# Melthizar/RRTE

Measured on AMD Instinct MI355X. Metric: Mray/s (primary+shadow) at 1920x1080, sdf-showcase scene; 1/2/4/8 GPU, higher is better.
Workload: dtype f32; 1 GPU; sdf-showcase 1920x1080, lambert_shadow, spp=1, max_depth=1, pixel-centre jitter; scene=sdf-showcase, width=1920, height=1080, mode=lambert_shadow, primary_rays_per_frame=2073600, frames_in_flight=4, hw_queues=32, parallelism=single

## Files before the change

### rrte_amd/abi.py

```python
from __future__ import annotations

import ctypes as C
import os
from pathlib import Path

import numpy as np

_HERE = Path(__file__).resolve().parent
LIB_PATH = Path(os.environ.get("RRTE_HIP_LIB", _HERE / "lib" / "librrte_hip.so"))

RRTE_OK, RRTE_INVALID_ARG, RRTE_HIP_ERROR, RRTE_RCCL_ERROR, RRTE_UNSUPPORTED_PRIM, RRTE_NO_DEVICE = range(6)
STATUS_NAMES = {0: "OK", 1: "INVALID_ARG", 2: "HIP_ERROR", 3: "RCCL_ERROR", 4: "UNSUPPORTED_PRIM", 5: "NO_DEVICE"}

PRIM_SPHERE, PRIM_PLANE, PRIM_TRIANGLE, PRIM_CUBE, PRIM_CYLINDER, PRIM_CONE, PRIM_CAPSULE, PRIM_SDF, PRIM_MESH = range(9)
PRIM_MESH_INSTANCE = 9
MAT_LAMBERTIAN, MAT_METAL, MAT_DIELECTRIC, MAT_EMISSIVE = range(4)
LIGHT_POINT, LIGHT_DIRECTIONAL, LIGHT_SPOT, LIGHT_AMBIENT = range(4)
PERSPECTIVE, ORTHOGRAPHIC = 0, 1
MODE_REFCOMPAT, MODE_LAMBERT_SHADOW = 0, 1
JITTER_CENTER, JITTER_RANDOM = 0, 1
ABI_VERSION = 2
FLAG_F32_LINEAR = 1
FLAG_GATHER_OVERLAP = 2

SDF_SPHERE, SDF_BOX, SDF_CYLINDER, SDF_PRISM, SDF_TORUS = 1, 2, 3, 4, 5
SDF_TUBE, SDF_RING, SDF_CONE, SDF_CAPSULE, SDF_ELLIPSOID = 6, 7, 8, 9, 10
SDF_UNION, SDF_DIFFERENCE, SDF_INTERSECTION = 32, 33, 34
SDF_SMOOTH_UNION, SDF_SMOOTH_DIFFERENCE, SDF_SMOOTH_INTERSECTION = 35, 36, 37
SDF_BEND, SDF_TWIST, SDF_TAPER, SDF_NOISE, SDF_WAVE = 64, 65, 66, 67, 68
SDF_POP_POINT = 96
SDF_MAX_STACK, SDF_MAX_POINT_STACK, SDF_MAX_OCTAVES = 8, 4, 8
UNIQUE_ID_BYTES = 128
JIT_OFF, JIT_ON, JIT_AUTO = 0, 1, 2
FPCHECK_SQRT, FPCHECK_RCP, FPCHECK_DIV, FPCHECK_SQRT_HW, FPCHECK_GAMMA_U8, FPCHECK_SQRT_BF = 0, 1, 2, 3, 4, 5


class Prim(C.Structure):
    _fields_ = [
        ("kind", C.c_uint32), ("material", C.c_int32), ("sdf_first", C.c_uint32), ("sdf_count", C.c_uint32),
        ("sdf_max_steps", C.c_uint32), ("sdf_step_scale", C.c_float), ("sdf_hit_eps", C.c_float),
        ("flags", C.c_uint32), ("p", C.c_float * 20), ("trs", C.c_float * 10), ("_pad", C.c_float * 10),
    ]


class Material(C.Structure):
    _fields_ = [("kind", C.c_uint32), ("fuzz", C.c_float), ("ior", C.c_float), ("_pad0", C.c_float),
                ("albedo", C.c_float * 4)]


class Light(C.Structure):
    _fields_ = [
        ("kind", C.c_uint32), ("intensity", C.c_float), ("range", C.c_float), ("linear", C.c_float),
        ("quadratic", C.c_float), ("inner_angle", C.c_float), ("outer_angle", C.c_float), ("_pad0", C.c_float),
        ("position", C.c_float * 4), ("direction", C.c_float * 4), ("color", C.c_float * 4),
    ]


class SdfNode(C.Structure):
    _fields_ = [("op", C.c_uint32), ("i", C.c_uint32 * 3), ("f", C.c_float * 12)]


class Camera(C.Structure):
    _fields_ = [
        ("position", C.c_float * 3), ("projection", C.c_uint32), ("rotation", C.c_float * 4),
        ("scale", C.c_float * 3), ("fov", C.c_float), ("aspect_ratio", C.c_float), ("near_plane", C.c_float),
        ("far_plane", C.c_float), ("left", C.c_float), ("right", C.c_float), ("bottom", C.c_float),
        ("top", C.c_float), ("_pad", C.c_float * 1),
    ]


class RenderParams(C.Structure):
    _fields_ = [
        ("width", C.c_uint32), ("height", C.c_uint32), ("samples_per_pixel", C.c_uint32),
        ("max_depth", C.c_uint32), ("mode", C.c_uint32), ("jitter", C.c_uint32), ("seed", C.c_uint32),
        ("flags", C.c_uint32), ("background", C.c_float * 4), ("t_min", C.c_float), ("shadow_bias", C.c_float),
        ("gamma", C.c_float), ("band_rows", C.c_uint32),
    ]


class MeshVertex(C.Structure):
    _fields_ = [("position", C.c_float * 3), ("normal", C.c_float * 3)]


class SceneIR(C.Structure):
    _fields_ = [
        ("prims", C.POINTER(Prim)), ("num_prims", C.c_uint32),
        ("materials", C.POINTER(Material)), ("num_materials", C.c_uint32),
        ("lights", C.POINTER(Light)), ("num_lights", C.c_uint32),
        ("sdf_nodes", C.POINTER(SdfNode)), ("num_sdf_nodes", C.c_uint32),
        ("camera", Camera),
        ("mesh_vertices", C.POINTER(MeshVertex)), ("num_mesh_vertices", C.c_uint32),
        ("mesh_indices", C.POINTER(C.c_uint32)), ("num_mesh_indices", C.c_uint32),
        ("mesh_version", C.c_uint64),
    ]


class Stats(C.Structure):
    _fields_ = [("primary_rays", C.c_uint64), ("shadow_rays", C.c_uint64), ("kernel_ms", C.c_double),
                ("gather_ms", C.c_double), ("upload_ms", C.c_double), ("frames", C.c_uint64),
                ("jit_active", C.c_uint32), ("hot_tiles", C.c_uint32), ("jit_compile_ms", C.c_double)]


assert C.sizeof(Prim) == 192 and C.sizeof(Material) == 32 and C.sizeof(Light) == 80
assert C.sizeof(SdfNode) == 64 and C.sizeof(Camera) == 80 and C.sizeof(RenderParams) == 64

_P = C.c_void_p
EXPORTS = {
    "rrte_hip_abi_version": (C.c_uint32, []),
    "rrte_hip_create": (C.c_int, [C.c_int, C.POINTER(_P)]),
    "rrte_hip_destroy": (None, [_P]),
    "rrte_hip_last_error": (C.c_char_p, [_P]),
    "rrte_hip_render": (C.c_int, [_P, C.POINTER(SceneIR), C.POINTER(RenderParams), _P]),
    "rrte_hip_render_f32": (C.c_int, [_P, C.POINTER(SceneIR), C.POINTER(RenderParams), _P, _P]),
    "rrte_hip_render_async": (C.c_int, [_P, C.POINTER(SceneIR), C.POINTER(RenderParams), _P, _P, _P]),
    "rrte_hip_synchronize": (C.c_int, [_P]),
    "rrte_hip_query": (C.c_int, [_P, C.POINTER(C.c_uint32)]),
    "rrte_hip_stats": (C.c_int, [_P, C.POINTER(Stats)]),
    "rrte_hip_set_jit": (C.c_int, [_P, C.c_int]),
    "rrte_hip_jit_check": (C.c_int, [C.POINTER(SceneIR), C.c_int, C.c_char_p, C.c_size_t]),
    "rrte_hip_fpcheck": (C.c_int, [C.c_int, C.c_int, C.c_uint64, C.c_uint64, C.POINTER(C.c_uint64)]),
    "rrte_hip_sdf_guards": (C.c_int, [C.POINTER(SdfNode), C.c_uint32, C.c_uint32, C.POINTER(SdfNode),
                                      C.POINTER(C.c_uint32)]),
    "rrte_hip_tile_order_plan": (C.c_int, [C.POINTER(C.c_uint32), C.c_uint32, C.c_uint32, C.POINTER(C.c_uint32),
                                           C.c_uint32, C.POINTER(C.c_uint32)]),
    "rrte_hip_jit_cache_key": (C.c_int, [C.c_char_p, C.c_char_p, C.c_char_p, C.c_size_t]),
    "rrte_hip_check_word": (C.c_int, [_P, C.POINTER(C.c_uint64)]),
    "rrte_hip_scene_dump": (C.c_int, [C.POINTER(SceneIR), C.POINTER(RenderParams), C.c_char_p]),
    "rrte_hip_scene_load": (C.c_int, [C.c_char_p, C.POINTER(SceneIR), C.POINTER(RenderParams), C.POINTER(_P)]),
    "rrte_hip_scene_free": (None, [_P]),
    "rrte_hip_comm_unique_id": (C.c_int, [_P]),
    "rrte_hip_comm_init": (C.c_int, [_P, C.c_int, C.c_int, _P]),
    "rrte_hip_render_gather": (C.c_int, [_P, C.POINTER(SceneIR), C.POINTER(RenderParams), C.c_int, _P]),
    "rrte_hip_render_gather_async": (C.c_int, [_P, C.POINTER(SceneIR), C.POINTER(RenderParams), C.c_int, _P, _P]),
    "rrte_hip_band_rows_for_rank": (C.c_uint32, [C.c_uint32, C.c_uint32, C.c_int, C.c_int]),
    "rrte_hip_band_layout": (C.c_int, [C.POINTER(SceneIR), C.POINTER(RenderParams), C.c_int, C.c_int,
                                       C.POINTER(C.c_uint32), C.POINTER(C.c_uint32), C.POINTER(C.c_uint32)]),
    "rrte_hip_band_rows_for_rank_ex": (C.c_uint32, [C.c_uint32, C.c_uint32, C.c_int, C.c_int, C.c_uint32, C.c_uint32,
                                                    C.c_uint32]),
    "rrte_hip_set_gather_batch": (C.c_int, [_P, C.c_uint32]),
    "rrte_hip_flush": (C.c_int, [_P]),
    "rrte_hip_gather_info": (C.c_int, [_P, C.POINTER(C.c_uint64), C.POINTER(C.c_uint32)]),
    "rrte_hip_build_id": (C.c_int, [C.c_char_p, C.c_size_t]),
    "rrte_hip_host_register": (C.c_int, [_P, C.c_void_p, C.c_size_t]),
    "rrte_hip_host_unregister": (C.c_int, [_P, C.c_void_p]),
    "rrte_hip_set_comm_timeout": (C.c_int, [_P, C.c_uint32]),
}

QUERY_CLOSEST, QUERY_ANY = 0, 1
QUERY_MAX_RAYS = 1 << 24


class Ray(C.Structure):
    _fields_ = [("origin", C.c_float * 3), ("t_min", C.c_float), ("direction", C.c_float * 3), ("t_max", C.c_float)]


class RayHit(C.Structure):
    _fields_ = [("t", C.c_float), ("prim", C.c_int32), ("point", C.c_float * 3), ("normal", C.c_float * 3),
                ("front_face", C.c_uint32), ("tri", C.c_uint32), ("material", C.c_int32), ("_pad", C.c_uint32)]


assert C.sizeof(Ray) == 32 and C.sizeof(RayHit) == 48

RAY_DTYPE = np.dtype([("origin", "<f4", (3,)), ("t_min", "<f4"), ("direction", "<f4", (3,)), ("t_max", "<f4")])
RAY_HIT_DTYPE = np.dtype([("t", "<f4"), ("prim", "<i4"), ("point", "<f4", (3,)), ("normal", "<f4", (3,)),
                          ("front_face", "<u4"), ("tri", "<u4"), ("material", "<i4"), ("_pad", "<u4")])
assert RAY_DTYPE.itemsize == 32 and RAY_HIT_DTYPE.itemsize == 48

QUERY_EXPORTS = {
    "rrte_hip_raycast": (C.c_int, [_P, C.POINTER(SceneIR), C.POINTER(Ray), C.c_uint32, C.c_uint32, C.POINTER(RayHit)]),
    "rrte_hip_raycast_async": (C.c_int, [_P, C.POINTER(SceneIR), _P, C.c_uint32, C.c_uint32, _P, _P]),
    "rrte_hip_pick": (C.c_int, [_P, C.POINTER(SceneIR), C.POINTER(RenderParams), C.POINTER(C.c_uint32), C.c_uint32,
                                C.POINTER(RayHit)]),
}

class MeshInfo(C.Structure):
    _fields_ = [("bvh_builds", C.c_uint64), ("ranges", C.c_uint32), ("tri_slots", C.c_uint32),
                ("bvh_nodes", C.c_uint32), ("_pad", C.c_uint32)]


assert C.sizeof(MeshInfo) == 24

MESH_EXPORTS = {
    "rrte_hip_mesh_info": (C.c_int, [_P, C.POINTER(MeshInfo)]),
}

class RefitInfo(C.Structure):
    _fields_ = [("refits", C.c_uint64), ("device_refits", C.c_uint64), ("levels", C.c_uint32),
                ("deformed", C.c_uint32)]


assert C.sizeof(RefitInfo) == 24

REFIT_EXPORTS = {
    "rrte_hip_mesh_refit": (C.c_int, [_P, C.POINTER(SceneIR)]),
    "rrte_hip_refit_info": (C.c_int, [_P, C.POINTER(RefitInfo)]),
    "rrte_hip_mesh_nodes": (C.c_int, [_P, C.c_void_p, C.c_size_t, C.POINTER(C.c_uint32)]),
    "rrte_hip_mesh_slots": (C.c_int, [_P, C.POINTER(C.c_uint32), C.c_size_t, C.POINTER(C.c_uint32)]),
}

MESH_BUILD_HOST, MESH_BUILD_DEVICE = 0, 1


class BuildInfo(C.Structure):
    _fields_ = [("device_builds", C.c_uint64), ("host_fallbacks", C.c_uint64), ("policy", C.c_uint32),
                ("depth", C.c_uint32)]


assert C.sizeof(BuildInfo) == 24

BUILD_EXPORTS = {
    "rrte_hip_set_mesh_build": (C.c_int, [_P, C.c_uint32]),
    "rrte_hip_build_info": (C.c_int, [_P, C.POINTER(BuildInfo)]),
}

SCENE_ACCEL_OFF, SCENE_ACCEL_ON = 0, 1
ACCEL_COUNT = 1
ACCEL_DEFAULT_MIN_PRIMS, ACCEL_MAX_PRIMS = 65, 16384


class AccelInfo(C.Structure):
    _fields_ = [("builds", C.c_uint64), ("fallbacks", C.c_uint64), ("searches", C.c_uint64),
                ("candidates", C.c_uint64), ("policy", C.c_uint32), ("min_prims", C.c_uint32),
                ("flags", C.c_uint32), ("nodes", C.c_uint32), ("depth", C.c_uint32), ("bounded", C.c_uint32),
                ("unbounded", C.c_uint32), ("reserved", C.c_uint32)]


assert C.sizeof(AccelInfo) == 64

ACCEL_EXPORTS = {
    "rrte_hip_set_scene_accel": (C.c_int, [_P, C.c_uint32, C.c_uint32, C.c_uint32]),
    "rrte_hip_accel_info": (C.c_int, [_P, C.POINTER(AccelInfo)]),
}

ENTRY_NONE, ENTRY_GENERIC, ENTRY_GENERAL, ENTRY_PLAIN = 0, 1, 2, 3

JIT_EXPORTS = {
    "rrte_hip_jit_entry": (C.c_int, [_P, C.POINTER(C.c_uint32)]),
    "rrte_hip_tile_rects": (C.c_int, [C.POINTER(SceneIR), C.POINTER(RenderParams), C.POINTER(C.c_uint32),
                                      C.POINTER(C.c_uint32), C.POINTER(C.c_uint32)]),
}

_lib = None


def load() -> C.CDLL:
    global _lib
    if _lib is not None:
        return _lib
    if not LIB_PATH.exists():
        raise RuntimeError(
            f"librrte_hip.so not found at {LIB_PATH}; build it with `python -c 'import __graft_entry__ as g; g.build()'`"
        )
    try:
        import torch
    except Exception:
        pass
    lib = C.CDLL(str(LIB_PATH), mode=C.RTLD_GLOBAL)
    for name, (res, args) in {**EXPORTS, **QUERY_EXPORTS, **MESH_EXPORTS, **REFIT_EXPORTS, **BUILD_EXPORTS,
                               **ACCEL_EXPORTS, **JIT_EXPORTS}.items():
        fn = getattr(lib, name)
        fn.restype = res
        fn.argtypes = args
    if lib.rrte_hip_abi_version() != ABI_VERSION:
        raise RuntimeError("librrte_hip.so ABI version mismatch")
    _lib = lib
    return lib


class RrteError(RuntimeError):
    def __init__(self, status: int, msg: str):
        super().__init__(f"rrte_hip {STATUS_NAMES.get(status, status)}: {msg}")
        self.status = status


def band_layout(scene_ref, params_ref, nranks: int, root: int = 0) -> tuple:
    sky, rb, pb = C.c_uint32(), C.c_uint32(), C.c_uint32()
    st = load().rrte_hip_band_layout(scene_ref, params_ref, nranks, root, C.byref(sky), C.byref(rb), C.byref(pb))
    if st != RRTE_OK:
        raise RuntimeError(f"rrte_hip_band_layout: status {st}")
    return sky.value, rb.value, pb.value


def build_id() -> str:
    buf = C.create_string_buffer(64)
    st = load().rrte_hip_build_id(buf, 64)
    if st != RRTE_OK:
        raise RuntimeError(f"rrte_hip_build_id: status {st}")
    return buf.value.decode()
```

### rrte_amd/csrc/jit.hip

```cpp
#include <hip/hip_runtime.h>
#include <hip/hiprtc.h>

#include <chrono>
#include <cinttypes>
#include <cstdio>
#include <cstdlib>
#include <cstring>
#include <mutex>
#include <sys/stat.h>
#include <unistd.h>
#include <string>
#include <vector>

#include "jit.hpp"

namespace rrte {
namespace {

struct JitHeader {
    const char* name;
    const char* text;
};
#include "jit_headers.inc"

void emit_f(std::string& s, float v) {
    char buf[48];
    if (v != v) {
        snprintf(buf, sizeof buf, "__builtin_nanf(\"\")");
    } else if (v == __builtin_huge_valf()) {
        snprintf(buf, sizeof buf, "__builtin_huge_valf()");
    } else if (v == -__builtin_huge_valf()) {
        snprintf(buf, sizeof buf, "(-__builtin_huge_valf())");
    } else {
        snprintf(buf, sizeof buf, "%af", (double)v);
    }
    s += buf;
}

void emit_fa(std::string& s, const float* v, int n) {
    s += "{";
    for (int i = 0; i < n; ++i) {
        if (i) s += ",";
        emit_f(s, v[i]);
    }
    s += "}";
}

void emit_u(std::string& s, uint32_t v) { s += std::to_string(v) + "u"; }

}

static std::string full_scene_arrays(const DPrim* prims, uint32_t np, const DMaterial* mats, uint32_t nm,
                                     const DLight* lights, uint32_t nl, const rrte_sdf_node* nodes, uint32_t nn);
static void append_kernel(std::string& s, const rrte_sdf_node* nodes, uint32_t nn, int mode, bool cull, bool single,
                          bool topo);

std::string jit_source(const DPrim* prims, uint32_t np, const DMaterial* mats, uint32_t nm, const DLight* lights,
                       uint32_t nl, const rrte_sdf_node* nodes, uint32_t nn, int mode, bool cull, bool single,
                       const JitTopo* topo) {
    std::string s;
    s.reserve(8192 + np * 600 + nn * 200);
    s += "typedef __hip_internal::uint8_t uint8_t;\ntypedef __hip_internal::uint32_t uint32_t;\n"
         "typedef __hip_internal::int32_t int32_t;\ntypedef __hip_internal::uint64_t uint64_t;\n"
         "#include \"ray_kernels.hpp\"\n#define RRTE_JIT_BLOCK 64\n"
         "namespace rrte_jit {\nstruct Scene {\n  static constexpr bool kStatic = true, kTopo = ";
    s += topo ? "true;\n" : "false;\n";
    s += "  static constexpr uint32_t num_prims = " + std::to_string(np) + "u, num_lights = " + std::to_string(nl) +
         "u, num_materials = " + std::to_string(nm) + "u;\n";
    if (topo) {
        s += "  static constexpr rrte::TopoPrim topo_prims[" + std::to_string(np ? np : 1) + "] = {";
        for (uint32_t i = 0; i < np; ++i) {
            s += i ? ",{" : "{";
            emit_u(s, prims[i].kind); s += ",";
            emit_u(s, prims[i].sdf_first); s += ",";
            emit_u(s, prims[i].sdf_count); s += ",";
            s += topo->convex[i] ? "true}" : "false}";
        }
        if (!np) s += "{}";
        s += "};\n  static constexpr rrte::TopoNode topo_nodes[" + std::to_string(nn ? nn : 1) + "] = {";
        for (uint32_t i = 0; i < nn; ++i) {
            s += i ? ",{" : "{";
            emit_u(s, nodes[i].op); s += ",{";
            emit_u(s, nodes[i].i[0]); s += ",";
            emit_u(s, nodes[i].i[1]); s += ",";
            emit_u(s, nodes[i].i[2]); s += "}}";
        }
        if (!nn) s += "{}";
        s += "};\n  static constexpr rrte::TopoLight topo_lights[" + std::to_string(nl ? nl : 1) + "] = {";
        for (uint32_t i = 0; i < nl; ++i) {
            s += i ? ",{" : "{";
            emit_u(s, lights[i].kind); s += ",";
            s += topo->cullable[i] ? "true}" : "false}";
        }
        if (!nl) s += "{}";
        s += "};\n  const rrte::DPrim* prims;\n  const rrte::DMaterial* mats;\n  const rrte::DLight* lights;\n"
             "  const rrte_sdf_node* nodes;\n";
    } else {
        s += full_scene_arrays(prims, np, mats, nm, lights, nl, nodes, nn);
    }
    s += "  rrte::MeshView mesh;  // runtime mesh buffers (kernel argument)\n};\n}  // namespace rrte_jit\n";
    s += "#include \"search_groups.hpp\"\n";
    append_kernel(s, nodes, nn, mode, cull, single, topo != nullptr);
    return s;
}

static std::string full_scene_arrays(const DPrim* prims, uint32_t np, const DMaterial* mats, uint32_t nm,
                              const DLight* lights, uint32_t nl, const rrte_sdf_node* nodes, uint32_t nn) {
    std::string s;
    s += "  static constexpr rrte::DPrim prims[" + std::to_string(np ? np : 1) + "] = {";
    for (uint32_t i = 0; i < np; ++i) {
        const DPrim& p = prims[i];
        s += i ? ",\n    {" : "\n    {";
        emit_u(s, p.kind); s += ",";
        s += std::to_string(p.material) + ",";
        emit_u(s, p.sdf_first); s += ",";
        emit_u(s, p.sdf_count); s += ",";
        emit_u(s, p.sdf_max_steps); s += ",";
        emit_f(s, p.sdf_step_scale); s += ",";
        emit_f(s, p.sdf_hit_eps); s += ",";
        emit_u(s, p.flags); s += ",";
        emit_fa(s, p.p, 20); s += ",";
        emit_fa(s, p.xf, 12); s += ",";
        emit_fa(s, p.inv, 12); s += ",{}}";
    }
    if (!np) s += "{}";
    s += "};\n  static constexpr rrte::DMaterial mats[" + std::to_string(nm ? nm : 1) + "] = {";
    for (uint32_t i = 0; i < nm; ++i) {
        const DMaterial& m = mats[i];
        s += i ? ",{" : "{";
        emit_u(s, m.kind); s += ",";
        emit_f(s, m.fuzz); s += ",";
        emit_f(s, m.ior); s += ",0.0f,";
        emit_fa(s, m.albedo, 4); s += "}";
    }
    if (!nm) s += "{}";
    s += "};\n  static constexpr rrte::DLight lights[" + std::to_string(nl ? nl : 1) + "] = {";
    for (uint32_t i = 0; i < nl; ++i) {
        const DLight& l = lights[i];
        s += i ? ",{" : "{";
        emit_u(s, l.kind); s += ",";
        const float sc[7] = {l.intensity, l.range, l.linear, l.quadratic, l.inner_angle, l.outer_angle, 0.0f};
        for (int k = 0; k < 7; ++k) { emit_f(s, sc[k]); s += ","; }
        emit_fa(s, l.position, 4); s += ",";
        emit_fa(s, l.direction, 4); s += ",";
        emit_fa(s, l.color, 4); s += ",";
        emit_fa(s, l.cI, 4); s += "}";
    }
    if (!nl) s += "{}";
    s += "};\n  static constexpr rrte_sdf_node nodes[" + std::to_string(nn ? nn : 1) + "] = {";
    for (uint32_t i = 0; i < nn; ++i) {
        const rrte_sdf_node& n = nodes[i];
        s += i ? ",{" : "{";
        emit_u(s, n.op); s += ",{";
        emit_u(s, n.i[0]); s += ",";
        emit_u(s, n.i[1]); s += ",";
        emit_u(s, n.i[2]); s += "},";
        emit_fa(s, n.f, 12); s += "}";
    }
    if (!nn) s += "{}";
    s += "};\n";
    return s;
}

static void append_kernel(std::string& s, const rrte_sdf_node* nodes, uint32_t nn, int mode, bool cull, bool single,
                   bool topo) {
    int min_waves = 8;
    if (const char* w = getenv("RRTE_JIT_MIN_WAVES"); w && *w) min_waves = atoi(w);
    std::string lb = "RRTE_JIT_BLOCK";
    if (min_waves > 0) lb += ", " + std::to_string(min_waves);
    auto entry = [&](const char* name, const char* traits) {
        s += "extern \"C\" __global__ __launch_bounds__(" + lb + ") void " + name + "(rrte::KParams kp, rrte::Cull cl, "
             "rrte::MeshView mv, uint32_t* __restrict__ o8, float4* __restrict__ of, unsigned long long* __restrict__ ctr, "
             "rrte::SceneValues sv) {\n"
             "  rrte::ray_kernel_body<" + std::to_string(mode) + ", rrte_jit::Scene, " + (single ? "true" : "false") + ", " +
             (cull ? "true" : "false") + ", " + traits + ">(kp, rrte_jit::Scene{" +
             (topo ? "sv.prims, sv.mats, sv.lights, sv.nodes, mv" : "mv") + "}, cl, o8, of, ctr);\n}\n";
    };
    entry("rrte_jit_kernel", "rrte::LaunchAny");
    if (single && !topo) entry("rrte_jit_kernel_plain", "rrte::LaunchPlain");
}

static std::vector<std::string> rtc_options() {
    std::vector<std::string> opts = {"--offload-arch=gfx950", "-O1", "-ffp-contract=off", "-std=c++17", "-Wno-pass-failed",
                                     "-mllvm", "-amdgpu-sched-strategy=max-ilp"};
    if (const char* e = getenv("RRTE_JIT_EXTRA_OPTS")) {
        std::string t;
        for (const char* c = e;; ++c) {
            if (*c == ' ' || *c == 0) {
                if (!t.empty()) opts.push_back(t);
                t.clear();
                if (*c == 0) break;
            } else {
                t += *c;
            }
        }
    }
    return opts;
}

static bool rtc_compile(const std::string& src, std::vector<char>& code, std::string& log) {
    if (const char* dump = getenv("RRTE_JIT_DUMP")) {
        if (FILE* f = fopen(dump, "w")) {
            fwrite(src.data(), 1, src.size(), f);
            fclose(f);
        }
    }
    static const std::vector<std::string> texts = [] {
        std::vector<std::string> v;
        for (const JitHeader& h : kJitHeaders) {
            std::string t = h.text;
            for (const JitHeader& o : kJitHeaders) {
                const std::string tail = std::string("/") + o.name + "\"";
                for (size_t end = t.find(tail); end != std::string::npos; end = t.find(tail, end + 1)) {
                    const size_t path = t.rfind('\n', end) + 1 + 10;
                    if (t.compare(path - 10, 10, "#include \"") == 0) t.erase(path, end + 1 - path);
                }
            }
            v.push_back(t);
        }
        return v;
    }();
    std::vector<const char*> hdrs, names;
    for (size_t i = 0; i < texts.size(); ++i) {
        hdrs.push_back(texts[i].c_str());
        names.push_back(kJitHeaders[i].name);
    }
    hiprtcProgram prog;
    if (hiprtcCreateProgram(&prog, src.c_str(), "rrte_scene_jit.hip", (int)hdrs.size(), hdrs.data(), names.data()) !=
        HIPRTC_SUCCESS) {
        log = "hiprtcCreateProgram failed";
        return false;
    }
    const std::vector<std::string> sopts = rtc_options();
    std::vector<const char*> opts;
    for (const std::string& o : sopts) opts.push_back(o.c_str());
    hiprtcResult r = hiprtcCompileProgram(prog, (int)opts.size(), opts.data());
    size_t ls = 0;
    hiprtcGetProgramLogSize(prog, &ls);
    if (ls > 1) {
        std::vector<char> l(ls + 1, 0);
        hiprtcGetProgramLog(prog, l.data());
        log.assign(l.data());
    }
    if (r != HIPRTC_SUCCESS) {
        hiprtcDestroyProgram(&prog);
        if (log.empty()) log = hiprtcGetErrorString(r);
        return false;
    }
    size_t cs = 0;
    hiprtcGetCodeSize(prog, &cs);
    code.resize(cs);
    hiprtcGetCode(prog, code.data());
    hiprtcDestroyProgram(&prog);
    return true;
}

bool jit_compile_only(const std::string& src, std::string& log) {
    std::vector<char> code;
    return rtc_compile(src, code, log);
}

namespace {

uint64_t fnv1a(const std::string& s, uint64_t h) {
    for (unsigned char c : s) {
        h ^= c;
        h *= 0x100000001b3ull;
    }
    return h;
}

std::string cache_dir() {
    if (const char* e = getenv("RRTE_JIT_CACHE"); e && e[0] == '0') return "";
    if (const char* d = getenv("RRTE_JIT_CACHE_DIR"); d && *d) return d;
    if (const char* x = getenv("XDG_CACHE_HOME"); x && *x) return std::string(x) + "/rrte-jit";
    if (const char* h = getenv("HOME"); h && *h) return std::string(h) + "/.cache/rrte-jit";
    return "";
}

struct CacheKey {
    uint64_t a, b, len;
    std::string name;
};

const std::string& headers_digest() {
    static const std::string d = [] {
        std::string all;
        for (const JitHeader& h : kJitHeaders) {
            all += h.text;
            all += '\0';
        }
        char buf[64];
        snprintf(buf, sizeof buf, "%016" PRIx64 "%016" PRIx64 ":%zu", fnv1a(all, 0xcbf29ce484222325ull),
                 fnv1a(all, 0x84222325cbf29ce4ull), all.size());
        return std::string(buf);
    }();
    return d;
}

}

std::string jit_cache_name(const std::string& src, const char* hdr_override);

namespace {

CacheKey cache_key(const std::string& src, const char* hdr_override = nullptr) {
    int maj = 0, min = 0;
    hiprtcVersion(&maj, &min);
    std::string all = src;
    all += "\n//headers:";
    if (hdr_override) all += std::to_string(fnv1a(hdr_override, 0xcbf29ce484222325ull));
    else all += headers_digest();
    all += "\n//opts:";
    for (const std::string& o : rtc_options()) {
        all += o;
        all += '\x1f';
    }
    all += "//hiprtc " + std::to_string(maj) + "." + std::to_string(min);
    CacheKey k{fnv1a(all, 0xcbf29ce484222325ull), fnv1a(all, 0x84222325cbf29ce4ull), (uint64_t)all.size(), ""};
    char buf[64];
    snprintf(buf, sizeof buf, "%016" PRIx64 "%016" PRIx64, k.a, k.b);
    k.name = buf;
    return k;
}

bool cache_load(const std::string& dir, const CacheKey& k, std::vector<char>& code) {
    FILE* f = fopen((dir + "/" + k.name + ".hsaco").c_str(), "rb");
    if (!f) return false;
    uint64_t hdr[4] = {};
    bool ok = fread(hdr, sizeof hdr, 1, f) == 1 && hdr[0] == k.a && hdr[1] == k.b && hdr[2] == k.len && hdr[3] > 0 &&
              hdr[3] < (256ull << 20);
    if (ok) {
        code.resize(hdr[3]);
        ok = fread(code.data(), 1, code.size(), f) == code.size();
    }
    fclose(f);
    return ok;
}

void cache_store(const std::string& dir, const CacheKey& k, const std::vector<char>& code) {
    std::string cur;
    for (size_t i = 0; i <= dir.size(); ++i) {
        if (i == dir.size() || dir[i] == '/') {
            if (!cur.empty()) (void)mkdir(cur.c_str(), 0755);
        }
        if (i < dir.size()) cur += dir[i];
    }
    const std::string tmp = dir + "/." + k.name + "." + std::to_string((long)getpid()) + ".tmp";
    FILE* f = fopen(tmp.c_str(), "wb");
    if (!f) return;
    const uint64_t hdr[4] = {k.a, k.b, k.len, (uint64_t)code.size()};
    const bool ok = fwrite(hdr, sizeof hdr, 1, f) == 1 && fwrite(code.data(), 1, code.size(), f) == code.size();
    if (fclose(f) == 0 && ok) (void)rename(tmp.c_str(), (dir + "/" + k.name + ".hsaco").c_str());
    else (void)remove(tmp.c_str());
}

}

std::string jit_cache_name(const std::string& src, const char* hdr_override) { return cache_key(src, hdr_override).name; }

JitCode jit_compile_code(const std::string& src) {
    static std::mutex mu;
    std::lock_guard<std::mutex> lock(mu);
    JitCode jc;
    const auto t0 = std::chrono::steady_clock::now();
    const std::string dir = cache_dir();
    const CacheKey key = cache_key(src);
    if (!dir.empty() && cache_load(dir, key, jc.code)) {
        jc.ok = true;
        jc.from_cache = true;
    } else {
        jc.ok = rtc_compile(src, jc.code, jc.log);
        if (jc.ok && !dir.empty()) cache_store(dir, key, jc.code);
    }
    jc.compile_ms = std::chrono::duration<double, std::milli>(std::chrono::steady_clock::now() - t0).count();
    return jc;
}

bool jit_load(const JitCode& jc, JitKernel& out, std::string& log) {
    if (!jc.ok) {
        log = jc.log;
        return false;
    }
    hipError_t e = hipModuleLoadData(&out.module, jc.code.data());
    if (e != hipSuccess) {
        log = std::string("hipModuleLoadData: ") + hipGetErrorString(e);
        return false;
    }
    e = hipModuleGetFunction(&out.fn, out.module, "rrte_jit_kernel");
    if (e != hipSuccess) {
        log = std::string("hipModuleGetFunction: ") + hipGetErrorString(e);
        (void)hipModuleUnload(out.module);
        out.module = nullptr;
        return false;
    }
    if (hipModuleGetFunction(&out.fn_plain, out.module, "rrte_jit_kernel_plain") != hipSuccess) {
        out.fn_plain = nullptr;
        (void)hipGetLastError();
    }
    out.code_bytes = jc.code.size();
    out.compile_ms = jc.compile_ms;
    out.from_cache = jc.from_cache;
    return true;
}

bool jit_compile(const std::string& src, JitKernel& out, std::string& log) {
    return jit_load(jit_compile_code(src), out, log);
}

void jit_release(JitKernel& k) {
    if (k.module) (void)hipModuleUnload(k.module);
    k.module = nullptr;
    k.fn = nullptr;
    k.fn_plain = nullptr;
}

}
```

Baseline: 124,800 Mray/s.

## Clip SDF sphere-CSG marching with conservative analytic bounding-sphere exit tests

For SDF primitives built from two spheres combined by a union, intersection or difference (plain or smooth), a conservative bound is computed at JIT time from padded sphere radii. Before sphere-tracing, the ray is tested against these bounds. Rays that miss are rejected, and t_max is tightened to the analytic exit distance, which aims to cut wasted march steps. The padding terms are meant to keep the bound conservative, but a float-error mistake could drop valid hits. A host query API is also added.

```diff
diff --git a/include/rrte_hip_clip.h b/include/rrte_hip_clip.h
--- /dev/null
+++ b/include/rrte_hip_clip.h
@@ -0,0 +1,31 @@
+#ifndef RRTE_HIP_CLIP_H
+#define RRTE_HIP_CLIP_H
+
+#include "rrte_hip.h"
+
+#ifdef __cplusplus
+extern "C" {
+#endif
+
+#define RRTE_CLIP_NONE         0u
+#define RRTE_CLIP_DIFFERENCE   1u
+#define RRTE_CLIP_INTERSECTION 2u
+#define RRTE_CLIP_UNION        4u
+
+typedef struct rrte_clip_info {
+    uint32_t cls;
+    float c1, c2;
+    float a_center[3];
+    float a_c0;
+    float b_center[3];
+    float b_c0;
+    uint32_t reserved;
+} rrte_clip_info;
+
+rrte_status rrte_hip_march_clip(const rrte_scene_ir* scene, uint32_t object, rrte_clip_info* out);
+
+#ifdef __cplusplus
+}
+#endif
+
+#endif
diff --git a/rrte_amd/abi.py b/rrte_amd/abi.py
--- a/rrte_amd/abi.py
+++ b/rrte_amd/abi.py
@@ -240,6 +240,20 @@
                                       C.POINTER(C.c_uint32), C.POINTER(C.c_uint32)]),
 }
 
+CLIP_NONE, CLIP_DIFFERENCE, CLIP_INTERSECTION, CLIP_UNION = 0, 1, 2, 4
+
+
+class ClipInfo(C.Structure):
+    _fields_ = [("cls", C.c_uint32), ("c1", C.c_float), ("c2", C.c_float), ("a_center", C.c_float * 3),
+                ("a_c0", C.c_float), ("b_center", C.c_float * 3), ("b_c0", C.c_float), ("reserved", C.c_uint32)]
+
+
+assert C.sizeof(ClipInfo) == 48
+
+CLIP_EXPORTS = {
+    "rrte_hip_march_clip": (C.c_int, [C.POINTER(SceneIR), C.c_uint32, C.POINTER(ClipInfo)]),
+}
+
 _lib = None
 
 
@@ -257,7 +271,7 @@
         pass
     lib = C.CDLL(str(LIB_PATH), mode=C.RTLD_GLOBAL)
     for name, (res, args) in {**EXPORTS, **QUERY_EXPORTS, **MESH_EXPORTS, **REFIT_EXPORTS, **BUILD_EXPORTS,
-                               **ACCEL_EXPORTS, **JIT_EXPORTS}.items():
+                               **ACCEL_EXPORTS, **JIT_EXPORTS, **CLIP_EXPORTS}.items():
         fn = getattr(lib, name)
         fn.restype = res
         fn.argtypes = args
diff --git a/rrte_amd/csrc/jit.hip b/rrte_amd/csrc/jit.hip
--- a/rrte_amd/csrc/jit.hip
+++ b/rrte_amd/csrc/jit.hip
@@ -22,6 +22,7 @@
     const char* text;
 };
 #include "jit_headers.inc"
+#include "march_clip.inc"
 
 void emit_f(std::string& s, float v) {
     char buf[48];
@@ -99,6 +100,7 @@
         s += full_scene_arrays(prims, np, mats, nm, lights, nl, nodes, nn);
     }
     s += "  rrte::MeshView mesh;  // runtime mesh buffers (kernel argument)\n};\n}  // namespace rrte_jit\n";
+    s += kMarchClipText;
     s += "#include \"search_groups.hpp\"\n";
     append_kernel(s, nodes, nn, mode, cull, single, topo != nullptr);
     return s;
diff --git a/rrte_amd/csrc/march_clip.hip b/rrte_amd/csrc/march_clip.hip
--- /dev/null
+++ b/rrte_amd/csrc/march_clip.hip
@@ -0,0 +1,34 @@
+#include "context.hpp"
+#include "sdf_guard.hpp"
+#include "../../include/rrte_hip_clip.h"
+
+#define RRTE_MARCH_CLIP_HOST 1
+#include "march_clip.hpp"
+
+using namespace rrte;
+
+extern "C" rrte_status rrte_hip_march_clip(const rrte_scene_ir* s, uint32_t object, rrte_clip_info* out) {
+    if (!s || !out || object >= s->num_prims || !s->prims || (s->num_sdf_nodes && !s->sdf_nodes)) return RRTE_INVALID_ARG;
+    if ((s->num_mesh_indices && !s->mesh_indices) || (s->num_mesh_vertices && !s->mesh_vertices)) return RRTE_INVALID_ARG;
+    std::vector<DPrim> prims;
+    std::vector<DMaterial> mats;
+    std::vector<DLight> lights;
+    lower_scene(s, prims, mats, lights);
+    const std::vector<rrte_sdf_node> nodes = decorate_scene_sdf(s, env_guard_setting());
+    *out = rrte_clip_info{};
+    const DPrim& pr = prims[object];
+    if (pr.kind == RRTE_PRIM_SDF && (uint64_t)pr.sdf_first + pr.sdf_count > nodes.size()) return RRTE_INVALID_ARG;
+#if RRTE_MARCH_CLIP
+    const clip::Info ci = clip::info(pr, nodes.data());
+    out->cls = ci.cls;
+    out->c1 = ci.c1;
+    out->c2 = ci.c2;
+    for (int j = 0; j < 3; ++j) {
+        out->a_center[j] = ci.a.c[j];
+        out->b_center[j] = ci.b.c[j];
+    }
+    out->a_c0 = ci.a.c0;
+    out->b_c0 = ci.b.c0;
+#endif
+    return RRTE_OK;
+}
diff --git a/rrte_amd/csrc/march_clip.hpp b/rrte_amd/csrc/march_clip.hpp
--- /dev/null
+++ b/rrte_amd/csrc/march_clip.hpp
@@ -0,0 +1,135 @@
+#ifndef RRTE_MARCH_CLIP
+#define RRTE_MARCH_CLIP 7
+#endif
+#if RRTE_MARCH_CLIP
+namespace rrte {
+namespace clip {
+
+constexpr uint32_t kDifference = 1u, kIntersection = 2u, kUnion = 4u;
+struct Part { float c[3]; float c0; };
+struct Info { uint32_t cls; float c1, c2; Part a, b; };
+
+constexpr bool bounded(float x) { return x > -0x1p40f && x < 0x1p40f; }
+constexpr float mag(float x) { return x < 0.0f ? -x : x; }
+constexpr float l1(const float* v) { return (mag(v[0]) + mag(v[1])) + mag(v[2]); }
+
+constexpr Info info(const DPrim& pr, const rrte_sdf_node* nodes) {
+    const Info none{};
+    if (pr.kind != RRTE_PRIM_SDF || pr.sdf_count != 3u) return none;
+    const rrte_sdf_node& A = nodes[pr.sdf_first];
+    const rrte_sdf_node& B = nodes[pr.sdf_first + 1u];
+    const rrte_sdf_node& O = nodes[pr.sdf_first + 2u];
+    if (A.op != RRTE_SDF_SPHERE || B.op != RRTE_SDF_SPHERE || O.op < RRTE_SDF_UNION || O.op > RRTE_SDF_SMOOTH_INTERSECTION)
+        return none;
+    if (A.i[2] != 0u || B.i[2] != 0u || O.i[2] != 0u) return none;
+    for (int j = 0; j < 7; ++j)
+        if (!bounded(A.f[j]) || !bounded(B.f[j])) return none;
+    for (int j = 0; j < 4; ++j)
+        if (!bounded(pr.p[j])) return none;
+    const bool smooth = O.op >= RRTE_SDF_SMOOTH_UNION;
+    const float k = smooth ? O.f[0] : 0.0f;
+    if (!bounded(O.f[0]) || (smooth && !(k > 0.0f))) return none;
+    const float eps = pr.sdf_hit_eps, R = pr.p[3];
+    if (!(A.f[3] >= 0.0f && B.f[3] >= 0.0f && R >= 0.0f && eps >= 0.0f && bounded(eps))) return none;
+    if (!(pr.sdf_step_scale > 0.0f && bounded(pr.sdf_step_scale))) return none;
+    const bool uni = O.op == RRTE_SDF_UNION || O.op == RRTE_SDF_SMOOTH_UNION;
+    const bool dif = O.op == RRTE_SDF_DIFFERENCE || O.op == RRTE_SDF_SMOOTH_DIFFERENCE;
+    Info r{};
+    r.cls = uni ? kUnion : dif ? kDifference : kIntersection;
+    constexpr float grow = 1.0f + 0x1p-10f;
+    const float EE = eps * (1.0f + 0x1p-20f) + 0x1p-17f;
+    float sa = 0.0f, sb = 0.0f;
+    for (int j = 0; j < 7; ++j) {
+        sa += mag(A.f[j]);
+        sb += mag(B.f[j]);
+    }
+    const float K = (sa > sb ? sa : sb) + mag(O.f[0]);
+    const float dconst = 0x1p-17f * ((l1(pr.p) + 4.0f * R) + K);
+    r.c1 = EE * 1.001f * grow;
+    r.c2 = (0x1p-17f + EE * 0x1p-8f) * grow;
+    const rrte_sdf_node* leaf[2] = {&A, &B};
+    Part* part[2] = {&r.a, &r.b};
+    for (int s = 0; s < 2; ++s) {
+        const float* f = leaf[s]->f;
+        const float off = (mag(f[0] - pr.p[0]) + mag(f[1] - pr.p[1])) + mag(f[2] - pr.p[2]);
+        const float kt = 1.002f * (off + R) + 0x1p-8f * (l1(pr.p) + l1(f));
+        for (int j = 0; j < 3; ++j) part[s]->c[j] = f[j];
+        part[s]->c0 = (((f[3] + (uni ? 0.25f * k : 0.0f)) + EE * kt) + dconst) * grow;
+    }
+    return r;
+}
+
+}
+}
+
+#ifndef RRTE_MARCH_CLIP_HOST
+namespace rrte {
+namespace clip {
+
+template <class S, uint32_t I>
+constexpr Info info_of() {
+    if constexpr (S::kTopo) return Info{};
+    else return info(S::prims[I], S::nodes);
+}
+
+template <class S, uint32_t I, bool SECOND>
+__device__ __forceinline__ void part_exit(const Ray& r, float o1, bool& miss, float& exit) {
+    constexpr Info ci = info_of<S, I>();
+    constexpr Part pt = SECOND ? ci.b : ci.a;
+    const f3 oc = vsub(r.o, V(pt.c[0], pt.c[1], pt.c[2]));
+    const float b = vdot(oc, r.d);
+    const float q = vdot(oc, oc);
+    const float rho = (pt.c0 + ci.c1 * fabsf(b)) + ci.c2 * o1;
+    const float rr = rho * rho;
+    const float du = (b * b - (q - rr)) + 0x1p-18f * (q + rr);
+    miss = du < 0.0f;
+    const float s = __builtin_amdgcn_sqrtf(du);
+    exit = (s - b) + 0x1p-17f * ((fabsf(b) + s) + rho);
+}
+
+template <class S, uint32_t I>
+__device__ __forceinline__ bool reach(const Ray& r, float t_min, float& t_max) {
+    constexpr Info ci = info_of<S, I>();
+    const bool unit = fabsf(vdot(r.d, r.d) - 1.0f) <= 0x1p-20f;
+    const float o1 = (fabsf(r.o.x) + fabsf(r.o.y)) + fabsf(r.o.z);
+    bool ma, mb = false;
+    float ea, eb, ex;
+    part_exit<S, I, false>(r, o1, ma, ea);
+    if constexpr (ci.cls == kDifference) {
+        ex = ea;
+    } else {
+        part_exit<S, I, true>(r, o1, mb, eb);
+        if constexpr (ci.cls == kIntersection) {
+            ex = mn(ea, eb);
+            ma = ma || mb;
+        } else {
+            const float both = (eb == eb) ? mx(ea, eb) : eb;
+            ex = ma ? eb : mb ? ea : both;
+            ma = ma && mb;
+        }
+    }
+    if (unit && (ma || ex < t_min)) return false;
+    t_max = (unit && ex < t_max) ? ex : t_max;
+    return true;
+}
+
+}
+
+template <bool NEED_HIT, uint32_t I, bool ANY = false>
+__device__ __forceinline__ bool intersect_at(const rrte_jit::Scene& sc, UC<I> ii, const Ray& r, float t_min, float t_max,
+                                             Hit& out) {
+    constexpr uint32_t cls = clip::info_of<rrte_jit::Scene, I>().cls;
+    if constexpr ((cls & (uint32_t)(RRTE_MARCH_CLIP)) != 0u) {
+        if (!clip::reach<rrte_jit::Scene, I>(r, t_min, t_max)) return false;
+    }
+    return intersect_at<NEED_HIT, rrte_jit::Scene, I, ANY>(sc, ii, r, t_min, t_max, out);
+}
+template <uint32_t I>
+__device__ __forceinline__ bool any_hit_at(const rrte_jit::Scene& sc, UC<I> ii, const Ray& r, float t_min, float t_max,
+                                           Hit& h) {
+    return intersect_at<false, I, true>(sc, ii, r, t_min, t_max, h);
+}
+
+}
+#endif
+#endif
```

Result: faster. 131,600 Mray/s, median of 6 (+5.5%).
